# Desilo/liberate-fhe

Measured on AMD Instinct MI355X. Metric: NTTs/sec (forward negacyclic poly-NTT, logN=16, L=30 limbs, bit-exact vs reference semantics), higher is better.
Workload: dtype int64; 1 GPU; gold preset (logN=16), rows 9..38 of the prime chain (25 scale + base + 4 special primes = 30 limbs), 128 polynomials per GPU per step, forward NTT via lf_ntt_ws (C ABI: lf_ntt through a resident workspace of the operands' size); workspace_bytes=2013511680, batch_per_gpu=128, limbs=30, logN=16, parallelism=replicas x1 (independent polynomials)

## Files before the change

liberate_fhe_amd/csrc/ckks_ntt_core.h:

```cpp
#pragma once
#include "ckks_common.h"
#include <stdlib.h>

#define NTT_THREADS 512
#define NTT_PASS_WAVES 6
#define NTT_LDS_WORDS ((1 << NTT_TILE_LOG_MAX) + (1 << (NTT_TILE_LOG_MAX - 3)))
#define TAIL_NONE (-1)
#define SMALL_PRIME_LIMIT (1ull << 41)

#define PAD(L) ((L) + ((L) >> 3))
#define PAD_STRIDE(LOGDL) ((1 << (LOGDL)) + ((1 << (LOGDL)) >> 3))
#define NTT_FLAG_WORD NTT_LDS_WORDS

namespace {

__device__ __forceinline__ int lf_tid() {
    const int wave = __builtin_amdgcn_readfirstlane((int)threadIdx.x >> 6);
    int lane;
    asm volatile("v_mbcnt_lo_u32_b32 %0, -1, 0\n\tv_mbcnt_hi_u32_b32 %0, -1, %0" : "=v"(lane));
    return (wave << 6) | lane;
}

__device__ __forceinline__ void lds_barrier() {
    asm volatile("s_waitcnt lgkmcnt(0)" ::: "memory");
// ... 935 lines not shown
    }
}

#ifndef NTT_COL_THREADS
#define NTT_COL_THREADS 128
#endif

template <class T>
__device__ __forceinline__ T *uniform_ptr(T *p) {
    typedef T __attribute__((address_space(1))) *GP;
    GP g = (GP)p;
    asm("" : "+s"(g));
    return (T *)g;
}

template <class T>
__device__ __forceinline__ T *uniform_at(T *p, unsigned i) {
    typedef T __attribute__((address_space(1))) *GP;
    typedef char __attribute__((address_space(1))) *GB;
    GP g = (GP)p;
    asm("" : "+s"(g));
    return (T *)(GP)((GB)g + (unsigned)(i * (unsigned)sizeof(T)));
}

__device__ __forceinline__ unsigned lane_here(unsigned i, const void *row) {
    asm("" : "+v"(i) : "s"(row));
    return i;
}

typedef long long ll2_t __attribute__((ext_vector_type(2)));
__device__ __forceinline__ longlong2 nt_load2(const i64 *p) {
    const ll2_t v = __builtin_nontemporal_load(reinterpret_cast<const ll2_t *>(p));
    longlong2 r;
    r.x = v.x, r.y = v.y;
    return r;
}
__device__ __forceinline__ void nt_store2(i64 *p, const longlong2 &v) {
    ll2_t t;
    t.x = v.x, t.y = v.y;
    __builtin_nontemporal_store(t, reinterpret_cast<ll2_t *>(p));
}
#define NT_EXACT true
#define NT_RLOAD true
#define NT_INV true
#define NT_KS_EXT true
#define NT_RSTORE false
#define NT_RCOLS false
#define COLS_LD_ALL(dst, ptr)                                                            \
    if (nt) {                                                                            \
        _Pragma("unroll") for (int k = 0; k < R; ++k) dst[k] = __builtin_nontemporal_load(ptr); \
    } else {                                                                             \
        _Pragma("unroll") for (int k = 0; k < R; ++k) dst[k] = *(ptr);                   \
    }
#define COLS_ST_ALL(ptr, val)                                                            \
    if (nt) {                                                                            \
        _Pragma("unroll") for (int k = 0; k < R; ++k) __builtin_nontemporal_store((i64)(val), ptr); \
    } else {                                                                             \
        _Pragma("unroll") for (int k = 0; k < R; ++k) *(ptr) = (val);                    \
    }
#define INV_LD(p) (NT_INV ? __builtin_nontemporal_load(p) : *(p))
#define INV_LD2(p) (NT_INV ? nt_load2(p) : *reinterpret_cast<const longlong2 *>(p))
#define INV_ST(p, v)                                              \
    do {                                                          \
        if (NT_INV) __builtin_nontemporal_store((i64)(v), p);     \
        else *(p) = (v);                                          \
    } while (0)

template <class A, int K>
__device__ __forceinline__ void cols_fwd_stages(typename A::T (&x)[1 << K], const Ctx &c) {
#pragma unroll
    for (int u = 0; u < K; ++u) {
        const int du = 1 << (K - 1 - u);
#pragma unroll
        for (int j = 0; j < (1 << u); ++j) {
            const int e0 = j << (K - u);
            const int idx = (1 << u) + j;
            const typename A::W wv = A::tw(c, idx);
#pragma unroll
            for (int t = 0; t < du; ++t) A::fwd(c, x[e0 + t], x[e0 + t + du], wv, idx);
        }
    }
}

#define LF_NTT_RS_MAX 8
struct RescaleSrc {
    const i64 *in[LF_NTT_RS_MAX];
    const i64 *row0[LF_NTT_RS_MAX];
    const i64 *scales;
    i64 round_at;
};

template <bool DP, int K, bool RS = false>
__device__ __forceinline__ void fwd_cols_body(int b, i64 *__restrict__ a, const PassGeom &g, const RowList &rl,
                                              const i64 *__restrict__ psi_br, const double *__restrict__ psi_dp,
                                              const i64 *__restrict__ Rs, const i64 *__restrict__ ql,
                                              const i64 *__restrict__ qh, const i64 *__restrict__ kl,
                                              const i64 *__restrict__ kh, const RescaleSrc *rsrc = nullptr) {
    constexpr int R = 1 << K;
    const int logC = g.logN - K;
    const int chunks = (1 << logC) / NTT_COL_THREADS;
    const int chunk = b % chunks, r = b / chunks;
    const int poly = __builtin_amdgcn_readfirstlane(r % g.batch), crow = __builtin_amdgcn_readfirstlane((int)rl.id[r / g.batch]);
    const bool enter = (Rs != nullptr) && !(DP && g.plain);

    Ctx c;
    c.m = load_mod(ql, qh, kl, kh, crow);
    c.tw_mont = psi_br + ((i64)crow << g.logN);
    set_aux<DP>(c, psi_dp, crow, g.logN);
    c.d = DP ? make_dp_tab(c.m, c.tw_dp) : make_dp(c.m);
    c.relaxed = g.relaxed;
    c.inv_reduce = 0;
    const i64 rs = enter ? Rs[crow] : 0;
    i64 *colu = a + ((i64)(poly * g.rows + crow) << g.logN) + chunk * NTT_COL_THREADS;
    const unsigned lane = threadIdx.x;
    const bool nt = g.relaxed ? NT_RCOLS : NT_EXACT;

    if (RS && DP && g.relaxed) {
        const i64 j = (i64)chunk * NTT_COL_THREADS + threadIdx.x;
        const i64 *src = rsrc->in[poly] + ((i64)crow << g.logN) + j;
        const i64 *z0 = rsrc->row0[poly] + j;
        i64 sp = redc62(rsrc->scales[crow], c.m.q, c.m.k);
        sp = sp < (i64)c.m.q ? sp : sp - (i64)c.m.q;
        const double scp = (double)sp;
        const double r1 = enter ? (double)((1ull << 62) % c.m.q) : 0.0;
        double x[R];
#pragma unroll
        for (int k = 0; k < R; ++k) {
            const i64 z = z0[(i64)k << logC];
            double v = dp_mulmod_bal(dp_from_signed(src[(i64)k << logC] - z), scp, c.d) + (z > rsrc->round_at ? 1.0 : 0.0);
            if (enter) v = dp_mulmod_bal(v, r1, c.d);
            x[k] = v;
        }
        cols_fwd_stages<ArithDpR, K>(x, c);
        if (g.pln & PLN_OUT) {
            i64 *rowb = a + ((i64)(poly * g.rows + crow) << g.logN);
            const i64 col0 = (i64)chunk * NTT_COL_THREADS;
            unsigned *lo = reinterpret_cast<unsigned *>(rowb) + col0;
            unsigned short *hi = reinterpret_cast<unsigned short *>(rowb + ((i64)1 << (g.logN - 1))) + col0;
#pragma unroll
            for (int k = 0; k < R; ++k) {
                const i64 o = dp_to_word(dp_reduce(x[k], c.d.q, c.d.qinv));
                __builtin_nontemporal_store((unsigned)o, uniform_at(lo + ((i64)k << logC), lane));
                __builtin_nontemporal_store((unsigned short)((u64)o >> 32), uniform_at(hi + ((i64)k << logC), lane));
            }
            return;
        }
        COLS_ST_ALL(uniform_at(colu + ((i64)k << logC), lane), dp_to_word(dp_reduce(x[k], c.d.q, c.d.qinv)))
        return;
    }
    i64 w[R];
    if (RS) {
        const i64 j = (i64)chunk * NTT_COL_THREADS + threadIdx.x;
        const i64 *src = rsrc->in[poly] + ((i64)crow << g.logN) + j;
        const i64 *z0 = rsrc->row0[poly] + j;
        const i64 sc = rsrc->scales[crow], qq = (i64)c.m.q;
#pragma unroll
        for (int k = 0; k < R; ++k) {
            const i64 z = z0[(i64)k << logC];
            const i64 v = mm62s(src[(i64)k << logC] - z, sc, c.m.q, c.m.k) + (i64)(z > rsrc->round_at);
            w[k] = v < qq ? v : v - qq;
        }
    } else {
        COLS_LD_ALL(w, uniform_at(colu + ((i64)k << logC), lane))
    }
    int odd = 0;
#pragma unroll
    for (int k = 0; k < R; ++k) {
        if (g.relaxed && !DP) w[k] = w[k] < 0 ? w[k] + c.m.q2 : w[k];
        odd |= ((u64)w[k] >= (u64)c.m.q2);
    }
    if (DP && (g.relaxed || !odd)) {
        double x[R];
        const double r1 = enter ? (double)((1ull << 62) % c.m.q) : 0.0;
#pragma unroll
        for (int k = 0; k < R; ++k) {
            double v = g.relaxed ? dp_from_signed(w[k]) : dp_from_word(w[k]);
            if (enter) {
                v = dp_mulmod(v, r1, c.d);
                if (!g.relaxed && dp_below_fix_limit(v)) v = dp_lazy_fix(v, (u64)w[k], (u64)rs, c.d.q);
            }
            x[k] = v;
        }
        if (g.relaxed) cols_fwd_stages<ArithDpR, K>(x, c);
        else cols_fwd_stages<ArithDp, K>(x, c);
        const double md = g.relaxed ? c.d.q : c.d.q2, mi = g.relaxed ? c.d.qinv : c.d.q2inv;
        COLS_ST_ALL(uniform_at(colu + ((i64)k << logC), lane), dp_to_word(dp_reduce(x[k], md, mi)))
    } else {
        if (enter) {
#pragma unroll
            for (int k = 0; k < R; ++k) {
                w[k] = mm62s(w[k], rs, c.m.q, c.m.k);
                odd |= ((u64)w[k] >= (u64)c.m.q2);
            }
        }
        if (!DP && g.relaxed) {
            cols_fwd_stages<ArithShoup, K>(w, c);
            COLS_ST_ALL(uniform_at(colu + ((i64)k << logC), lane), ArithShoup::canon(c, w[k]))
            return;
        }
        if (odd || DP) cols_fwd_stages<ArithInt<true>, K>(w, c);
        else cols_fwd_stages<ArithInt<false>, K>(w, c);
        COLS_ST_ALL(uniform_at(colu + ((i64)k << logC), lane), w[k])
    }
}

template <bool DP, int K>
__device__ __forceinline__ void fwd_cols_ws_body(int b, const i64 *__restrict__ a, i64 *__restrict__ ws,
                                                 unsigned char *__restrict__ wflags, const PassGeom &g, const RowList &rl,
                                                 const i64 *__restrict__ psi_br, const double *__restrict__ psi_dp,
                                                 const i64 *__restrict__ Rs, const i64 *__restrict__ ql,
                                                 const i64 *__restrict__ qh, const i64 *__restrict__ kl,
                                                 const i64 *__restrict__ kh) {
    constexpr int R = 1 << K;
    const int logC = g.logN - K;
    const int chunks = (1 << logC) / NTT_COL_THREADS;
    const int chunk = b % chunks, r = b / chunks;
    const int poly = __builtin_amdgcn_readfirstlane(r % g.batch), crow = __builtin_amdgcn_readfirstlane((int)rl.id[r / g.batch]);
    const bool enter = Rs != nullptr;
    Ctx c;
    c.m = load_mod(ql, qh, kl, kh, crow);
    c.tw_mont = psi_br + ((i64)crow << g.logN);
    set_aux<DP>(c, psi_dp, crow, g.logN);
    c.d = DP ? make_dp_tab(c.m, c.tw_dp) : make_dp(c.m);
    c.relaxed = 0;
    c.inv_reduce = 0;
    const i64 rs = enter ? Rs[crow] : 0;
    const i64 ri = (i64)(poly * g.rows + crow);
    const i64 col0 = (i64)chunk * NTT_COL_THREADS;
    const i64 *colu = a + (ri << g.logN) + col0;
    const unsigned lane = threadIdx.x;
    i64 w[R];
#pragma unroll
    for (int k = 0; k < R; ++k) w[k] = __builtin_nontemporal_load(uniform_at(colu + ((i64)k << logC), lane));
    int odd = 0;
#pragma unroll
    for (int k = 0; k < R; ++k) odd |= ((u64)w[k] >= (u64)c.m.q2);
    if (DP && !odd) {
        double x[R];
        const double r1 = enter ? (double)((1ull << 62) % c.m.q) : 0.0;
#pragma unroll
        for (int k = 0; k < R; ++k) {
            double v = dp_from_word(w[k]);
            if (enter) {
                v = dp_mulmod(v, r1, c.d);
                if (dp_below_fix_limit(v)) v = dp_lazy_fix(v, (u64)w[k], (u64)rs, c.d.q);
            }
            x[k] = v;
        }
        cols_fwd_stages<ArithDp, K>(x, c);
#pragma unroll
        for (int k = 0; k < R; ++k) w[k] = dp_to_word(dp_reduce(x[k], c.d.q2, c.d.q2inv));
    } else {
        if (enter) {
#pragma unroll
            for (int k = 0; k < R; ++k) {
                w[k] = mm62s(w[k], rs, c.m.q, c.m.k);
                odd |= ((u64)w[k] >= (u64)c.m.q2);
            }
        }
        if (odd || DP) cols_fwd_stages<ArithInt<true>, K>(w, c);
        else cols_fwd_stages<ArithInt<false>, K>(w, c);
    }
    i64 *orow = ws + (ri << g.logN);
    const bool wide = __builtin_amdgcn_ballot_w64(odd != 0) != 0;
    if ((lane & 63u) == 0) {
        const unsigned c0 = (unsigned)col0 + lane;
        wflags[(ri << 6) + (((c0 >> 6) & 3u) << 4) + (c0 >> 8)] = wide ? 1 : 0;
    }
    if constexpr (!DP) {
        const unsigned ls = lane_here(lane, orow);
#pragma unroll
        for (int k = 0; k < R; ++k) __builtin_nontemporal_store(w[k], uniform_at(orow + col0 + ((i64)k << logC), ls));
    } else {
        unsigned *lo = reinterpret_cast<unsigned *>(orow) + col0;
        unsigned short *mid = reinterpret_cast<unsigned short *>(orow + ((i64)1 << (g.logN - 1))) + col0;
#pragma unroll
        for (int k = 0; k < R; ++k) __builtin_nontemporal_store((unsigned)w[k], uniform_at(lo + ((i64)k << logC), lane));
#pragma unroll
        for (int k = 0; k < R; ++k)
            __builtin_nontemporal_store((unsigned short)((u64)w[k] >> 32), uniform_at(mid + ((i64)k << logC), lane));
        if (wide) {
            unsigned short *top = reinterpret_cast<unsigned short *>(orow + 3 * ((i64)1 << (g.logN - 2))) + col0;
#pragma unroll
            for (int k = 0; k < R; ++k) top[((i64)k << logC) + lane] = (unsigned short)((u64)w[k] >> 48);
        }
    }
}

template <int K>
__global__ void __launch_bounds__(NTT_COL_THREADS) ntt_fwd_cols_ws(const i64 *__restrict__ a, i64 *__restrict__ ws,
                                                                  unsigned char *__restrict__ wflags, PassGeom g, ClassLists cl,
                                                                  const i64 *__restrict__ psi_br,
                                                                  const double *__restrict__ psi_dp,
                                                                  const i64 *__restrict__ Rs, const i64 *__restrict__ ql,
                                                                  const i64 *__restrict__ qh, const i64 *__restrict__ kl,
                                                                  const i64 *__restrict__ kh) {
    const int b = blockIdx.x;
    if (b < cl.in_blocks) {
        if (b < cl.in_real) fwd_cols_ws_body<false, K>(b, a, ws, wflags, g, cl.in, psi_br, psi_dp, Rs, ql, qh, kl, kh);
    } else {
        fwd_cols_ws_body<true, K>(b - cl.in_blocks, a, ws, wflags, g, cl.dp, psi_br, psi_dp, Rs, ql, qh, kl, kh);
    }
}

template <bool DP, int K>
__global__ void __launch_bounds__(NTT_COL_THREADS) ntt_fwd_cols(i64 *__restrict__ a, PassGeom g, RowList rl,
                                                               const i64 *__restrict__ psi_br,
                                                               const double *__restrict__ psi_dp, const i64 *__restrict__ Rs,
                                                               const i64 *__restrict__ ql, const i64 *__restrict__ qh,
                                                               const i64 *__restrict__ kl, const i64 *__restrict__ kh) {
    fwd_cols_body<DP, K>(blockIdx.x, a, g, rl, psi_br, psi_dp, Rs, ql, qh, kl, kh);
}

template <int K>
__global__ void __launch_bounds__(NTT_COL_THREADS) ntt_fwd_cols_mixed(i64 *__restrict__ a, PassGeom g, ClassLists cl,
                                                                     const i64 *__restrict__ psi_br,
                                                                     const double *__restrict__ psi_dp,
                                                                     const i64 *__restrict__ Rs, const i64 *__restrict__ ql,
                                                                     const i64 *__restrict__ qh, const i64 *__restrict__ kl,
                                                                     const i64 *__restrict__ kh) {
    const int b = blockIdx.x;
    if (b < cl.in_blocks) {
        if (b < cl.in_real) fwd_cols_body<false, K>(b, a, g, cl.in, psi_br, psi_dp, Rs, ql, qh, kl, kh);
    } else {
        fwd_cols_body<true, K>(b - cl.in_blocks, a, g, cl.dp, psi_br, psi_dp, Rs, ql, qh, kl, kh);
    }
}

template <int K>
__global__ void __launch_bounds__(NTT_COL_THREADS) ntt_fwd_cols_mixed_rs(i64 *__restrict__ a, PassGeom g, ClassLists cl,
                                                                        RescaleSrc rsrc, const i64 *__restrict__ psi_br,
                                                                        const double *__restrict__ psi_dp,
                                                                        const i64 *__restrict__ Rs, const i64 *__restrict__ ql,
                                                                        const i64 *__restrict__ qh, const i64 *__restrict__ kl,
                                                                        const i64 *__restrict__ kh) {
    const int b = blockIdx.x;
    if (b < cl.in_blocks) {
        if (b < cl.in_real) fwd_cols_body<false, K, true>(b, a, g, cl.in, psi_br, psi_dp, Rs, ql, qh, kl, kh, &rsrc);
    } else {
        fwd_cols_body<true, K, true>(b - cl.in_blocks, a, g, cl.dp, psi_br, psi_dp, Rs, ql, qh, kl, kh, &rsrc);
    }
}

template <bool DP, bool RLX>
__device__ __forceinline__ void inv_pass_body(i64 *sm, int b, const i64 *src, i64 *dst, const PassGeom &g0, const RowList &rl,
                                              const i64 *__restrict__ ipsi_br, const double *__restrict__ ipsi_dp,
                                              const i64 *__restrict__ Ninv, int tail, const i64 *__restrict__ ql,
// ... 417 lines not shown
```

liberate_fhe_amd/csrc/ckks_ntt_tile16.h:

```cpp
#pragma once
#include "ckks_ntt_core.h"

#define NTT16_THREADS 256
#define PAD16(L) ((L) + ((L) >> 4))
#define NTT16_LDS_WORDS (4096 + 256)
#define NTT16_FLAG NTT16_LDS_WORDS

namespace {

template <class A>
struct Tw16Early {
    typename A::W w1[1], w2[2], w4[4];
    __device__ __forceinline__ void load(const Ctx &c, int i) {
        A::tw_group(c, i, 1, w1);
        A::tw_group(c, i << 1, 2, w2);
        A::tw_group(c, i << 2, 4, w4);
    }
    __device__ __forceinline__ void get(int cnt, typename A::W (&wv)[8]) const {
#pragma unroll
        for (int j = 0; j < 4; ++j)
            if (j < cnt) wv[j] = cnt == 1 ? w1[0] : (cnt == 2 ? w2[j & 1] : w4[j]);
    }
};

// ... 262 lines not shown
    }
    if (CHECK) {
        int odd = 0;
#pragma unroll
        for (int e = 0; e < 16; ++e) odd |= ((u64)raw[e] >= (u64)c.m.q2);
        wave_flag_set16(sm, odd, w);
    }
    i64 o[16];
    bool ok;
    if constexpr (DP) {
        typedef typename DpArith<RLX>::type AD;
        double x[16];
#pragma unroll
        for (int e = 0; e < 16; ++e) x[e] = PLN ? dp_from_planes(plo[e], phi[e]) : RLX ? dp_from_signed(raw[e]) : dp_from_word(raw[e]);
        ok = fwd_tile16_steps<AD, true, RLX>(reinterpret_cast<double *>(sm), sm, x, w, base, E, s, c, CHECK, lastC);
        const double md = RLX ? c.d.q : c.d.q2, mi = RLX ? c.d.qinv : c.d.q2inv;
#pragma unroll
        for (int e = 0; e < 16; ++e) o[e] = dp_to_word(dp_reduce(x[e], md, mi));
    } else if constexpr (RLX) {
        ok = fwd_tile16_steps<ArithShoup, false, true>(sm, sm, raw, w, base, E, s, c, false, lastC);
#pragma unroll
        for (int e = 0; e < 16; ++e) o[e] = ArithShoup::canon(c, raw[e]);
    } else {
        ok = fwd_tile16_steps<ArithInt<false>, false, RLX>(sm, sm, raw, w, base, E, s, c, true, lastC);
#pragma unroll
        for (int e = 0; e < 16; ++e) o[e] = raw[e];
    }
    if (!ok) {
        __syncthreads();
        tile16_slow(sm, row + base, row + base, base, s, E, false, c);
        return;
    }
    if constexpr (PLN) {
        const int lane = w & 63, wave = w >> 6;
        unsigned *sw = reinterpret_cast<unsigned *>(sm + 17 * 64 * wave);
#pragma unroll
        for (int k = 0; k < 4; ++k) {
            const lf_u4_t v = {(unsigned)o[4 * k], (unsigned)o[4 * k + 1], (unsigned)o[4 * k + 2], (unsigned)o[4 * k + 3]};
            *reinterpret_cast<lf_u4_t *>(sw + lane * 20 + 4 * k) = v;
        }
#pragma unroll
        for (int k = 0; k < 2; ++k) {
            lf_u4_t v;
#pragma unroll
            for (int m = 0; m < 4; ++m)
                v[m] = (unsigned)(o[8 * k + 2 * m] >> 32) | ((unsigned)(o[8 * k + 2 * m + 1] >> 32) << 16);
            *reinterpret_cast<lf_u4_t *>(sw + 1280 + lane * 12 + 4 * k) = v;
        }
        wave_lds_sync();
        unsigned *lo = reinterpret_cast<unsigned *>(row) + base + (wave << 10);
        unsigned *hi = reinterpret_cast<unsigned *>(row + ((i64)1 << (E - 1))) + ((base + (wave << 10)) >> 1);
#pragma unroll
        for (int i = 0; i < 4; ++i) {
            const lf_u4_t v = *reinterpret_cast<const lf_u4_t *>(sw + (16 * i + (lane >> 2)) * 20 + 4 * (lane & 3));
            *reinterpret_cast<lf_u4_t *>(lo + (i << 8) + 4 * lane) = v;
        }
#pragma unroll
        for (int i = 0; i < 2; ++i) {
            const lf_u4_t v = *reinterpret_cast<const lf_u4_t *>(sw + 1280 + (32 * i + (lane >> 1)) * 12 + 4 * (lane & 1));
            *reinterpret_cast<lf_u4_t *>(hi + (i << 8) + 4 * lane) = v;
        }
        return;
    }
    {
        i64 *sp = sm + 17 * w;
#pragma unroll
        for (int e = 0; e < 16; ++e) sp[e] = o[e];
    }
    wave_lds_sync();
    const int L0 = ((w >> 6) << 10) + ((w & 63) << 1);
    const i64 *so = sm + PAD16(L0);
#pragma unroll
    for (int i = 0; i < 8; ++i) {
        longlong2 v;
        v.x = so[i * 136];
        v.y = so[i * 136 + 1];
        if constexpr (NTS) nt_store2(row + base + L0 + (i << 7), v);
        else *reinterpret_cast<longlong2 *>(row + base + L0 + (i << 7)) = v;
    }
}

template <bool DP, bool SKIP0>
__device__ __forceinline__ bool ws_load_tile(const i64 *__restrict__ srow, const unsigned char *__restrict__ wf, int base, int E,
                                             int w, i64 (&raw)[16]) {
    const int wave = __builtin_amdgcn_readfirstlane(w >> 6);
    w = (int)lane_here((unsigned)w, srow);
    const u64 *fp = reinterpret_cast<const u64 *>(wf + (wave << 4));
    const u64 fl = fp[0], fh = SKIP0 ? fp[0] : fp[1];
    if constexpr (DP) {
        const unsigned *lo = reinterpret_cast<const unsigned *>(srow) + base;
        const unsigned short *mid = reinterpret_cast<const unsigned short *>(srow + ((i64)1 << (E - 1))) + base;
#pragma unroll
        for (int e = 0; e < 16; ++e) {
            const unsigned l = __builtin_nontemporal_load(uniform_at(lo + (e << 8), (unsigned)w));
            const unsigned m = __builtin_nontemporal_load(uniform_at(mid + (e << 8), (unsigned)w));
            raw[e] = (i64)(((u64)m << 32) | (u64)l);
        }
        if ((fl | fh) != 0) {
            const unsigned short *top = reinterpret_cast<const unsigned short *>(srow + 3 * ((i64)1 << (E - 2))) + base;
#pragma unroll
            for (int e = 0; e < 16; ++e)
                if ((((e < 8 ? fl : fh) >> (8 * (e & 7))) & 0xffull) != 0) raw[e] |= (i64)((u64)top[(e << 8) + w] << 48);
        }
    } else {
#pragma unroll
        for (int e = 0; e < 16; ++e) raw[e] = __builtin_nontemporal_load(uniform_at(srow + base + (e << 8), (unsigned)w));
    }
    return (fl | fh) != 0;
}

template <bool DP, bool SKIP0>
__device__ __forceinline__ void fwd_tile16_ws(i64 *sm, const i64 *__restrict__ srow, const unsigned char *__restrict__ wf,
                                              i64 *__restrict__ row, int tile, const PassGeom &g, const Ctx &c,
                                              const Tw16Last<typename FwdArith<DP, false>::type> *lastC = nullptr) {
    const int w = lf_tid();
    const int base = tile << 12, E = g.logN, s = g.s0;
    i64 raw[16];
    const bool flagged = ws_load_tile<DP, SKIP0>(srow, wf, base, E, w, raw);
    {
        int odd = 0;
        if (flagged) {
#pragma unroll
            for (int e = 0; e < 16; ++e) odd |= ((u64)raw[e] >= (u64)c.m.q2);
        }
        wave_flag_set16(sm, odd, w);
    }
    i64 o[16];
    bool ok;
    if constexpr (DP) {
        double x[16];
#pragma unroll
        for (int e = 0; e < 16; ++e) x[e] = dp_from_word(raw[e]);
        ok = fwd_tile16_steps<ArithDp, true, false, SKIP0 ? 1 : 0>(reinterpret_cast<double *>(sm), sm, x, w, base, E, s, c, true, lastC);
#pragma unroll
        for (int e = 0; e < 16; ++e) o[e] = dp_to_word(dp_reduce(x[e], c.d.q2, c.d.q2inv));
    } else {
        ok = fwd_tile16_steps<ArithInt<false>, false, false, SKIP0 ? 1 : 0>(sm, sm, raw, w, base, E, s, c, true, lastC);
#pragma unroll
        for (int e = 0; e < 16; ++e) o[e] = raw[e];
    }
    if (!ok) {
        __syncthreads();
        ws_load_tile<DP, SKIP0>(srow, wf, base, E, w, raw);
#pragma unroll
        for (int e = 0; e < 16; ++e) sm[PAD16(w + (e << 8))] = raw[e];
        __syncthreads();
        tile16_slow_lds(sm, row + base, base, s, E, false, c, SKIP0 ? 1 : 0);
        return;
    }
    {
        i64 *sp = sm + 17 * w;
#pragma unroll
        for (int e = 0; e < 16; ++e) sp[e] = o[e];
    }
    wave_lds_sync();
    const int L0 = ((w >> 6) << 10) + ((w & 63) << 1);
    const i64 *so = sm + PAD16(L0);
#pragma unroll
    for (int i = 0; i < 8; ++i) {
        longlong2 v;
        v.x = so[i * 136];
        v.y = so[i * 136 + 1];
        if constexpr (NT_EXACT) nt_store2(row + base + L0 + (i << 7), v);
        else *reinterpret_cast<longlong2 *>(row + base + L0 + (i << 7)) = v;
    }
}

template <class A, bool DP, bool RLX>
__device__ __forceinline__ bool inv_tile16_steps(typename A::T *smt, const i64 *sm, typename A::T (&x)[16], int w, int base,
                                                 int logN, int s, const Ctx &c, bool check) {
    constexpr bool EX = DP && !RLX;
    const int iC = (1 << (logN - s - 4)) + ((base + 16 * w) >> (s + 4));
    const int pB = ((w >> 4) << 8) | (w & 15);
    const int iB = (1 << (logN - s - 8)) + ((base + pB) >> (s + 8));
    const int iA = (1 << (logN - s - 12)) + (base >> (s + 12));
    Tw16Early<A> twB;
    inv_step16<A, EX>(x, iC, c, nullptr);
    {
        typename A::T *sp = smt + 17 * w;
#pragma unroll
        for (int e = 0; e < 16; ++e) sp[e] = x[e];
    }
    twB.load(c, iB);
    lds_barrier();
    if (check && tile_flagged16(sm)) return false;
    {
        typename A::T *sp = smt + PAD16(pB);
#pragma unroll
        for (int e = 0; e < 16; ++e) x[e] = sp[e * 17];
        inv_step16<A, EX>(x, iB, c, &twB);
#pragma unroll
        for (int e = 0; e < 16; ++e) sp[e * 17] = x[e];
    }
    lds_barrier();
    {
        const typename A::T *sp = smt + PAD16(w);
#pragma unroll
        for (int e = 0; e < 16; ++e) x[e] = sp[e * 272];
    }
    inv_step16<A, EX>(x, iA, c, nullptr);
    return true;
}

template <bool DP, bool RLX, bool MUL = false, int PLN = 0>
__device__ __forceinline__ void inv_tile16(i64 *sm, const i64 *src_row, i64 *dst_row, int tile, const PassGeom &g, const Ctx &c,
                                           const i64 *mul_row = nullptr) {
    static_assert(!MUL || RLX, "product-on-load exists for the relaxed inverse transform only");
    static_assert(!PLN || (DP && RLX), "planes: relaxed fp64-class rows only");
    const int w = lf_tid();
    const int base = tile << 12, logN = g.logN, s = g.s0;
    constexpr bool CHECK = !RLX;
    const int L0 = ((w >> 6) << 10) + ((w & 63) << 1);
    if constexpr ((PLN & PLN_IN) != 0) {
        const int L4 = ((w >> 6) << 10) + ((w & 63) << 2);
        const unsigned *lo = reinterpret_cast<const unsigned *>(src_row) + base + L4;
        const unsigned *hi = reinterpret_cast<const unsigned *>(src_row + ((i64)1 << (logN - 1))) + ((base + L4) >> 1);
        lf_u4_t l[4], lb[4];
        lf_u2_t h[4], hb[4];
#pragma unroll
        for (int i = 0; i < 4; ++i) {
            l[i] = __builtin_nontemporal_load(reinterpret_cast<const lf_u4_t *>(lo + (i << 8)));
            h[i] = __builtin_nontemporal_load(reinterpret_cast<const lf_u2_t *>(hi + (i << 7)));
        }
        if (MUL) {
            const unsigned *mlo = reinterpret_cast<const unsigned *>(mul_row) + base + L4;
            const unsigned *mhi = reinterpret_cast<const unsigned *>(mul_row + ((i64)1 << (logN - 1))) + ((base + L4) >> 1);
// ... 335 lines not shown

template <bool DP, bool RLX>
__device__ __forceinline__ void seq16_loop(i64 *sm, i64 *dst, const PassGeom &g, const RowList &rl, int b0, int bend, int tpb,
                                           const i64 *__restrict__ tw_br, const double *__restrict__ tw_dp,
                                           const i64 *__restrict__ ql, const i64 *__restrict__ qh,
                                           const i64 *__restrict__ kl, const i64 *__restrict__ kh) {
    typedef typename FwdArith<DP, RLX>::type AC;
    const int w = lf_tid();
    Tw16Last<AC> last;
    int last_crow = -1, last_tile = -1;
    for (int i = 0; i < tpb; ++i) {
        const int b = b0 + 8 * i;
        const TileAt t = tile_at(g, rl, b, b < bend);
        if (!t.live) break;
        Ctx c;
        c.m = load_mod(ql, qh, kl, kh, t.crow);
        c.tw_mont = tw_br + ((i64)t.crow << g.logN);
        set_aux<DP>(c, tw_dp, t.crow, g.logN);
        c.d = DP ? make_dp_tab(c.m, c.tw_dp) : make_dp(c.m);
        c.relaxed = RLX ? 1 : 0;
        c.inv_reduce = 0;
        if (t.crow != last_crow || t.tile != last_tile) {
            last.load(c, (1 << (g.s0 + 8)) + (((t.tile << 12) + 16 * w) >> (g.logN - g.s0 - 8)));
            last_crow = t.crow, last_tile = t.tile;
        }
        if (i) lds_barrier();
        fwd_tile16<DP, RLX>(sm, dst + ((i64)(t.poly * g.rows + t.crow) << g.logN), t.tile, g, c, &last);
    }
}

template <bool RLX>
__global__ void __launch_bounds__(NTT16_THREADS, 4) ntt_pass16_fwd_seq(i64 *dst, PassGeom g, ClassLists cl, int total, int tpb,
                                                                         const i64 *__restrict__ tw_br,
                                                                         const double *__restrict__ tw_dp,
                                                                         const i64 *__restrict__ ql, const i64 *__restrict__ qh,
                                                                         const i64 *__restrict__ kl, const i64 *__restrict__ kh) {
    __shared__ i64 sm[NTT16_LDS_WORDS + 1];
    const int vb0 = (int)(blockIdx.x & 7) + 8 * (int)(blockIdx.x >> 3) * tpb;
    if (vb0 < cl.in_blocks) seq16_loop<false, RLX>(sm, dst, g, cl.in, vb0, cl.in_real, tpb, tw_br, tw_dp, ql, qh, kl, kh);
    else seq16_loop<true, RLX>(sm, dst, g, cl.dp, vb0 - cl.in_blocks, total - cl.in_blocks, tpb, tw_br, tw_dp, ql, qh, kl, kh);
}

template <bool DP> struct TilePf;
template <> struct TilePf<true> {
    unsigned lo[16];
    unsigned short mid[16];
};
template <> struct TilePf<false> {
    i64 raw[16];
};

template <bool DP, bool SKIP0>
__device__ __forceinline__ bool ws_prefetch_tile(const i64 *__restrict__ srow, const unsigned char *__restrict__ wf, int base, int E, int w,
                                                 TilePf<DP> &pf) {
    const int wave = __builtin_amdgcn_readfirstlane(w >> 6);
    w = (int)lane_here((unsigned)w, srow);
    const u64 *fp = reinterpret_cast<const u64 *>(wf + (wave << 4));
    const u64 fl = fp[0], fh = SKIP0 ? fp[0] : fp[1];
    if constexpr (DP) {
        const unsigned *lo = reinterpret_cast<const unsigned *>(srow) + base;
        const unsigned short *mid = reinterpret_cast<const unsigned short *>(srow + ((i64)1 << (E - 1))) + base;
#pragma unroll
        for (int e = 0; e < 16; ++e) {
            pf.lo[e] = __builtin_nontemporal_load(uniform_at(lo + (e << 8), (unsigned)w));
            pf.mid[e] = __builtin_nontemporal_load(uniform_at(mid + (e << 8), (unsigned)w));
        }
    } else {
#pragma unroll
        for (int e = 0; e < 16; ++e) pf.raw[e] = __builtin_nontemporal_load(uniform_at(srow + base + (e << 8), (unsigned)w));
    }
    return (fl | fh) != 0;
}

template <bool DP, bool SKIP0>
__device__ __forceinline__ void fwd_tile16_ws_pf(i64 *sm, TilePf<DP> &pf, bool &pf_flagged, const i64 *__restrict__ srow,
                                                  const unsigned char *__restrict__ wf, i64 *__restrict__ row, int tile,
                                                  const PassGeom &g, const Ctx &c, const Tw16Last<typename FwdArith<DP, false>::type> *lastC,
                                                  const i64 *__restrict__ nsrow, const unsigned char *__restrict__ nwf, int ntile) {
    const int w = lf_tid();
    const int base = tile << 12, E = g.logN, s = g.s0;
    i64 raw[16];
    const bool flagged = pf_flagged;
    if (flagged) {
        ws_load_tile<DP, SKIP0>(srow, wf, base, E, w, raw);
    } else if constexpr (DP) {
#pragma unroll
        for (int e = 0; e < 16; ++e) raw[e] = (i64)(((u64)pf.mid[e] << 32) | (u64)pf.lo[e]);
    } else {
#pragma unroll
        for (int e = 0; e < 16; ++e) raw[e] = pf.raw[e];
    }
    {
        int odd = 0;
        if (flagged) {
#pragma unroll
            for (int e = 0; e < 16; ++e) odd |= ((u64)raw[e] >= (u64)c.m.q2);
        }
        wave_flag_set16(sm, odd, w);
    }
    i64 o[16];
    bool ok;
    if constexpr (DP) {
        double x[16];
#pragma unroll
        for (int e = 0; e < 16; ++e) x[e] = dp_from_word(raw[e]);
        ok = fwd_tile16_steps<ArithDp, true, false, SKIP0 ? 1 : 0>(reinterpret_cast<double *>(sm), sm, x, w, base, E, s, c, true, lastC);
#pragma unroll
        for (int e = 0; e < 16; ++e) o[e] = dp_to_word(dp_reduce(x[e], c.d.q2, c.d.q2inv));
    } else {
        ok = fwd_tile16_steps<ArithInt<false>, false, false, SKIP0 ? 1 : 0>(sm, sm, raw, w, base, E, s, c, true, lastC);
#pragma unroll
        for (int e = 0; e < 16; ++e) o[e] = raw[e];
    }
    if (!ok) {
        __syncthreads();
        ws_load_tile<DP, SKIP0>(srow, wf, base, E, w, raw);
#pragma unroll
        for (int e = 0; e < 16; ++e) sm[PAD16(w + (e << 8))] = raw[e];
        __syncthreads();
        tile16_slow_lds(sm, row + base, base, s, E, false, c, SKIP0 ? 1 : 0);
        if (ntile >= 0) pf_flagged = ws_prefetch_tile<DP, SKIP0>(nsrow, nwf, ntile << 12, E, w, pf);
        else pf = TilePf<DP>{};
        return;
    }

    {
        i64 *sp = sm + 17 * w;
#pragma unroll
        for (int e = 0; e < 16; ++e) sp[e] = o[e];
    }
    __builtin_amdgcn_sched_barrier(0);
    if (ntile >= 0) pf_flagged = ws_prefetch_tile<DP, SKIP0>(nsrow, nwf, ntile << 12, E, w, pf);
    else pf = TilePf<DP>{};
    __builtin_amdgcn_sched_barrier(0);
    wave_lds_sync();
    const int L0 = ((w >> 6) << 10) + ((w & 63) << 1);
    const i64 *so = sm + PAD16(L0);
#pragma unroll
    for (int i = 0; i < 8; ++i) {
        longlong2 v;
        v.x = so[i * 136];
        v.y = so[i * 136 + 1];
        if constexpr (NT_EXACT) nt_store2(row + base + L0 + (i << 7), v);
        else *reinterpret_cast<longlong2 *>(row + base + L0 + (i << 7)) = v;
    }
}

#ifndef NTT16_WS_PREFETCH
#define NTT16_WS_PREFETCH 1
#endif

template <bool DP, bool SKIP0>
__device__ __forceinline__ void seq16_loop_ws(i64 *sm, const i64 *ws, const unsigned char *wflags, i64 *dst, const PassGeom &g,
                                              const RowList &rl, int b0, int bend, int tpb, const i64 *__restrict__ tw_br,
                                              const double *__restrict__ tw_dp, const i64 *__restrict__ ql,
                                              const i64 *__restrict__ qh, const i64 *__restrict__ kl, const i64 *__restrict__ kh) {
    typedef typename FwdArith<DP, false>::type AC;
    const int w = lf_tid();
    Tw16Last<AC> last;
    int last_crow = -1, last_tile = -1;
#if NTT16_WS_PREFETCH
    TilePf<DP> pf;
    bool pf_flagged = false;
    TileAt t = tile_at(g, rl, b0, b0 < bend);
    if (!t.live) return;
    {
        const i64 ri = (i64)(t.poly * g.rows + t.crow);
        pf_flagged = ws_prefetch_tile<DP, SKIP0>(ws + (ri << g.logN), wflags + (ri << 6), t.tile << 12, g.logN, w, pf);
    }
    for (int i = 0; i < tpb; ++i) {
        const int bn = b0 + 8 * (i + 1);
        TileAt tn = tile_at(g, rl, bn, i + 1 < tpb && bn < bend);
        Ctx c;
        c.m = load_mod(ql, qh, kl, kh, t.crow);
        c.tw_mont = tw_br + ((i64)t.crow << g.logN);
        set_aux<DP>(c, tw_dp, t.crow, g.logN);
        c.d = DP ? make_dp_tab(c.m, c.tw_dp) : make_dp(c.m);
        c.relaxed = 0;
        c.inv_reduce = 0;
        if (t.crow != last_crow || t.tile != last_tile) {
            last.load(c, (1 << (g.s0 + 8)) + (((t.tile << 12) + 16 * w) >> (g.logN - g.s0 - 8)));
            last_crow = t.crow, last_tile = t.tile;
        }
        if (i) lds_barrier();
        const i64 ri = (i64)(t.poly * g.rows + t.crow), rn = (i64)(tn.poly * g.rows + tn.crow);
        fwd_tile16_ws_pf<DP, SKIP0>(sm, pf, pf_flagged, ws + (ri << g.logN), wflags + (ri << 6), dst + (ri << g.logN), t.tile, g, c, &last,
                                    ws + (rn << g.logN), wflags + (rn << 6), tn.live ? tn.tile : -1);
        if (!tn.live) break;
        t = tn;
    }
#else
    for (int i = 0; i < tpb; ++i) {
        const int b = b0 + 8 * i;
        const TileAt t = tile_at(g, rl, b, b < bend);
        if (!t.live) break;
        Ctx c;
        c.m = load_mod(ql, qh, kl, kh, t.crow);
        c.tw_mont = tw_br + ((i64)t.crow << g.logN);
        set_aux<DP>(c, tw_dp, t.crow, g.logN);
// ... 163 lines not shown
```

Measured before the change: 82500 poly-NTT/s.

## Add stagewise exact DP column butterflies and store unreduced words to workspace

Replaces the generic double-precision column butterfly stages with a stagewise version. It batches the twiddle products in groups of eight and runs a wave-uniform check for the rare lazy-fix correction, so the fix-up path is skipped in the common case. When a wave has no wide values, the column pass also skips the final modular reduction. It writes the value plus a magic offset straight into the workspace, and the tile16 pass reduces these words later, but only on its flagged or slow reload path. This removes per-element reduction work in the first pass, at the cost of more complex correctness invariants around the unreduced representation.

```diff
diff --git a/liberate_fhe_amd/csrc/ckks_ntt_core.h b/liberate_fhe_amd/csrc/ckks_ntt_core.h
--- a/liberate_fhe_amd/csrc/ckks_ntt_core.h
+++ b/liberate_fhe_amd/csrc/ckks_ntt_core.h
@@ -1041,6 +1041,64 @@
     }
 }
 
+#ifndef LF_COLS_STAGEWISE
+#define LF_COLS_STAGEWISE 1
+#endif
+#ifndef LF_WS_UNREDUCED
+#define LF_WS_UNREDUCED 1
+#endif
+
+template <int K>
+__device__ __forceinline__ void cols_fwd_stages_exact(double (&x)[1 << K], const Ctx &c) {
+    constexpr int H = 1 << (K - 1);
+    constexpr int G = H < 8 ? H : 8;
+#pragma unroll
+    for (int u = 0; u < K; ++u) {
+        const int du = 1 << (K - 1 - u);
+#pragma unroll
+        for (int g0 = 0; g0 < H; g0 += G) {
+            double V[G];
+#pragma unroll
+            for (int i = 0; i < G; ++i) {
+                const int p = g0 + i, j = p >> (K - 1 - u), t = p & (du - 1);
+                V[i] = dp_mulmod(x[(j << (K - u)) + t + du], ArithDp::tw(c, (1 << u) + j), c.d);
+            }
+            int hmin = __double2hiint(V[0]);
+#pragma unroll
+            for (int i = 1; i < G; i += 2) {
+                if (i + 1 < G) hmin = min(min(hmin, __double2hiint(V[i])), __double2hiint(V[i + 1]));
+                else hmin = min(hmin, __double2hiint(V[i]));
+            }
+            if (__builtin_expect(__builtin_amdgcn_ballot_w64(hmin < 0x41500000) != 0, 0)) {
+#pragma unroll
+                for (int i = 0; i < G; ++i) {
+                    const int p = g0 + i, j = p >> (K - 1 - u), t = p & (du - 1);
+                    if (dp_below_fix_limit(V[i]))
+                        V[i] = dp_lazy_fix(V[i], (u64)c.tw_mont[(1 << u) + j],
+                                           (u64)dp_reduce(x[(j << (K - u)) + t + du], c.d.q2, c.d.q2inv), c.d.q);
+                }
+            }
+#pragma unroll
+            for (int i = 0; i < G; ++i) {
+                const int p = g0 + i, j = p >> (K - 1 - u), t = p & (du - 1);
+                const int ea = (j << (K - u)) + t;
+                const double U = x[ea], Vv = V[i];
+                x[ea] = U + Vv;
+                x[ea + du] = U - Vv;
+            }
+        }
+    }
+}
+
+template <int K>
+__device__ __forceinline__ void cols_fwd_stages_dp(double (&x)[1 << K], const Ctx &c) {
+#if LF_COLS_STAGEWISE
+    cols_fwd_stages_exact<K>(x, c);
+#else
+    cols_fwd_stages<ArithDp, K>(x, c);
+#endif
+}
+
 #define LF_NTT_RS_MAX 8
 struct RescaleSrc {
     const i64 *in[LF_NTT_RS_MAX];
@@ -1141,7 +1199,8 @@
             x[k] = v;
         }
         if (g.relaxed) cols_fwd_stages<ArithDpR, K>(x, c);
-        else cols_fwd_stages<ArithDp, K>(x, c);
+        else if constexpr (RS) cols_fwd_stages<ArithDp, K>(x, c);
+        else cols_fwd_stages_dp<K>(x, c);
         const double md = g.relaxed ? c.d.q : c.d.q2, mi = g.relaxed ? c.d.qinv : c.d.q2inv;
         COLS_ST_ALL(uniform_at(colu + ((i64)k << logC), lane), dp_to_word(dp_reduce(x[k], md, mi)))
     } else {
@@ -1194,6 +1253,8 @@
     int odd = 0;
 #pragma unroll
     for (int k = 0; k < R; ++k) odd |= ((u64)w[k] >= (u64)c.m.q2);
+    bool wide = false;
+    if constexpr (DP) wide = __builtin_amdgcn_ballot_w64(odd != 0) != 0;
     if (DP && !odd) {
         double x[R];
         const double r1 = enter ? (double)((1ull << 62) % c.m.q) : 0.0;
@@ -1206,9 +1267,15 @@
             }
             x[k] = v;
         }
-        cols_fwd_stages<ArithDp, K>(x, c);
-#pragma unroll
-        for (int k = 0; k < R; ++k) w[k] = dp_to_word(dp_reduce(x[k], c.d.q2, c.d.q2inv));
+        cols_fwd_stages_dp<K>(x, c);
+        if (LF_WS_UNREDUCED && !wide) {
+            const double off = DP_MAGIC + (double)K * c.d.q2;
+#pragma unroll
+            for (int k = 0; k < R; ++k) w[k] = __double_as_longlong(x[k] + off);
+        } else {
+#pragma unroll
+            for (int k = 0; k < R; ++k) w[k] = dp_to_word(dp_reduce(x[k], c.d.q2, c.d.q2inv));
+        }
     } else {
         if (enter) {
 #pragma unroll
@@ -1221,7 +1288,7 @@
         else cols_fwd_stages<ArithInt<false>, K>(w, c);
     }
     i64 *orow = ws + (ri << g.logN);
-    const bool wide = __builtin_amdgcn_ballot_w64(odd != 0) != 0;
+    if constexpr (!DP) wide = __builtin_amdgcn_ballot_w64(odd != 0) != 0;
     if ((lane & 63u) == 0) {
         const unsigned c0 = (unsigned)col0 + lane;
         wflags[(ri << 6) + (((c0 >> 6) & 3u) << 4) + (c0 >> 8)] = wide ? 1 : 0;
diff --git a/liberate_fhe_amd/csrc/ckks_ntt_tile16.h b/liberate_fhe_amd/csrc/ckks_ntt_tile16.h
--- a/liberate_fhe_amd/csrc/ckks_ntt_tile16.h
+++ b/liberate_fhe_amd/csrc/ckks_ntt_tile16.h
@@ -368,7 +368,7 @@
 
 template <bool DP, bool SKIP0>
 __device__ __forceinline__ bool ws_load_tile(const i64 *__restrict__ srow, const unsigned char *__restrict__ wf, int base, int E,
-                                             int w, i64 (&raw)[16]) {
+                                             int w, i64 (&raw)[16], const RowDp &d, bool redo = false) {
     const int wave = __builtin_amdgcn_readfirstlane(w >> 6);
     w = (int)lane_here((unsigned)w, srow);
     const u64 *fp = reinterpret_cast<const u64 *>(wf + (wave << 4));
@@ -382,11 +382,15 @@
             const unsigned m = __builtin_nontemporal_load(uniform_at(mid + (e << 8), (unsigned)w));
             raw[e] = (i64)(((u64)m << 32) | (u64)l);
         }
-        if ((fl | fh) != 0) {
+        if ((fl | fh) != 0 || (LF_WS_UNREDUCED && redo)) {
             const unsigned short *top = reinterpret_cast<const unsigned short *>(srow + 3 * ((i64)1 << (E - 2))) + base;
 #pragma unroll
-            for (int e = 0; e < 16; ++e)
+            for (int e = 0; e < 16; ++e) {
                 if ((((e < 8 ? fl : fh) >> (8 * (e & 7))) & 0xffull) != 0) raw[e] |= (i64)((u64)top[(e << 8) + w] << 48);
+#if LF_WS_UNREDUCED
+                else raw[e] = dp_to_word(dp_reduce(dp_from_word(raw[e]), d.q2, d.q2inv));
+#endif
+            }
         }
     } else {
 #pragma unroll
@@ -402,7 +406,7 @@
     const int w = lf_tid();
     const int base = tile << 12, E = g.logN, s = g.s0;
     i64 raw[16];
-    const bool flagged = ws_load_tile<DP, SKIP0>(srow, wf, base, E, w, raw);
+    const bool flagged = ws_load_tile<DP, SKIP0>(srow, wf, base, E, w, raw, c.d);
     {
         int odd = 0;
         if (flagged) {
@@ -427,7 +431,7 @@
     }
     if (!ok) {
         __syncthreads();
-        ws_load_tile<DP, SKIP0>(srow, wf, base, E, w, raw);
+        ws_load_tile<DP, SKIP0>(srow, wf, base, E, w, raw, c.d, true);
 #pragma unroll
         for (int e = 0; e < 16; ++e) sm[PAD16(w + (e << 8))] = raw[e];
         __syncthreads();
@@ -929,7 +933,7 @@
     i64 raw[16];
     const bool flagged = pf_flagged;
     if (flagged) {
-        ws_load_tile<DP, SKIP0>(srow, wf, base, E, w, raw);
+        ws_load_tile<DP, SKIP0>(srow, wf, base, E, w, raw, c.d);
     } else if constexpr (DP) {
 #pragma unroll
         for (int e = 0; e < 16; ++e) raw[e] = (i64)(((u64)pf.mid[e] << 32) | (u64)pf.lo[e]);
@@ -961,7 +965,7 @@
     }
     if (!ok) {
         __syncthreads();
-        ws_load_tile<DP, SKIP0>(srow, wf, base, E, w, raw);
+        ws_load_tile<DP, SKIP0>(srow, wf, base, E, w, raw, c.d, true);
 #pragma unroll
         for (int e = 0; e < 16; ++e) sm[PAD16(w + (e << 8))] = raw[e];
         __syncthreads();
```

New measurement: 82470 poly-NTT/s, median of 2. No clear change (-0.0%).
